# kevalmorabia97/CoVA-Web-Object-Detection

Measured on AMD Instinct MI355X. Metric: webpages/sec fwd+bwd (90 bboxes, K=24), higher is better.
Workload: dtype f32

## Files before the change

cova-web-object-detection_amd/_build.py:

```python
import glob
import os
import subprocess

PKG_DIR = os.path.dirname(os.path.abspath(__file__))
LIB_PATH = os.path.join(PKG_DIR, "lib", "libcova_hip.so")
SOURCES = sorted(glob.glob(os.path.join(PKG_DIR, "csrc", "*.hip")))
HEADERS = sorted(glob.glob(os.path.join(PKG_DIR, "csrc", "*.h")))


def needs_build():
    if not os.path.exists(LIB_PATH):
        return True
    t = os.path.getmtime(LIB_PATH)
    return any(os.path.getmtime(s) > t for s in SOURCES + HEADERS)


FILE_FLAGS = {"conv_wino.hip": ["-fno-slp-vectorize"],
              "conv_wgrad4.hip": ["-fno-slp-vectorize"]}


def build(force=False, verbose=False):
    if not force and not needs_build():
        return LIB_PATH
    hipcc = os.environ.get("HIPCC", "/opt/rocm/bin/hipcc")
    os.makedirs(os.path.dirname(LIB_PATH), exist_ok=True)
    objdir = os.path.join(PKG_DIR, "lib", "obj")
    os.makedirs(objdir, exist_ok=True)
    common = [hipcc, "--offload-arch=gfx950", "-O3", "-std=c++17", "-fPIC", "-fvisibility=hidden",
              "-Wall", "-Wno-unused-function"]
    common += os.environ.get("COVA_EXTRA_FLAGS", "").split()
    if os.environ.get("COVA_ABLATE"):
        common.append("-DCOVA_ABLATE=1")
    procs, objs = [], []
    for src in SOURCES:
        obj = os.path.join(objdir, os.path.basename(src)[:-4] + ".o")
        cmd = common + FILE_FLAGS.get(os.path.basename(src), []) + ["-c", src, "-o", obj]
        if verbose:
            print(" ".join(cmd))
        procs.append((cmd, subprocess.Popen(cmd)))
        objs.append(obj)
    for cmd, p in procs:
        if p.wait() != 0:
            raise subprocess.CalledProcessError(p.returncode, cmd)
    link = [hipcc, "--offload-arch=gfx950", "-shared", "-fPIC"] + objs + ["-o", LIB_PATH]
    if verbose:
        print(" ".join(link))
    subprocess.check_call(link)
    return LIB_PATH


if __name__ == "__main__":
    print(build(force=True, verbose=True))
```

cova-web-object-detection_amd/csrc/conv.hip:

```cpp
#include "common.h"
#include <stdlib.h>
#include "bf3.h"
#include "bn_tail.h"
#include <utility>
#include <type_traits>

namespace {

struct BnBwdEpi {
    const float *act, *z, *mean, *invstd;
};

__device__ __forceinline__ void epilogue_store_stats(const f32x16 &acc0, const f32x16 &acc1,
                                                     float *__restrict__ out,
                                                     const float *__restrict__ addend,
                                                     size_t pix_row_base, int x0, int W,
                                                     bool row_valid, int lane, float &s0,
                                                     float &s1, float &q0, float &q1,
                                                     const BnBwdEpi bn = BnBwdEpi{nullptr, nullptr,
                                                                                  nullptr, nullptr})
{
    const int li = lane & 31;
    s0 = s1 = q0 = q1 = 0.f;
    float mu0 = 0.f, mu1 = 0.f, is0 = 0.f, is1 = 0.f;
// ... 1075 lines not shown
                        const int ph = P0 + k, cph = ph < pool.H2 ? ph : pool.H2 - 1;
#pragma unroll
                        for (int e = 0; e <= par; ++e) {
                            const int pwc = W0 + e, cpw = pwc < pool.W2 ? pwc : pool.W2 - 1;
                            const unsigned o = (unsigned)((cph * pool.W2 + cpw) * 64 + c4 * 4);
                            o_.dpv[par][k][e] = *reinterpret_cast<const f32x4 *>(db + o);
                            o_.cdv[par][k][e] = *reinterpret_cast<const uint32_t *>(ib + o);
                            ok |= (ph < pool.H2 && pwc < pool.W2) ? (1u << (4 + 4 * par + 2 * k + e)) : 0u;
                        }
                    }
                }
            }
            o_.ok = ok;
        };
        auto finish = [&](const Ops &o_, uint32_t *dst) {
            if (WG1R_ABL & 4) return;
            const unsigned ok = o_.ok;
#pragma unroll
            for (int par = 0; par < 2; ++par) {
                const int kx0 = par ? 2 : 1;
                float d[2][4];
#pragma unroll
                for (int rr = 0; rr < 2; ++rr) {
                    float g[4] = {0.f, 0.f, 0.f, 0.f};
                    if (POOL) {
#pragma unroll
                        for (int k = 0; k < 2; ++k) {
                            if (rr == 0 && k == 1) continue;
                            const uint32_t ky = rr == 0 ? 1u : (k == 0 ? 2u : 0u);
#pragma unroll
                            for (int e = 0; e <= par; ++e) {
                                const uint32_t code = ky * 3u + (e == 0 ? (uint32_t)kx0 : 0u);
                                const bool win = (ok >> (4 + 4 * par + 2 * k + e)) & 1u;
#pragma unroll
                                for (int jx = 0; jx < 4; ++jx)
                                    g[jx] += (win && ((o_.cdv[par][k][e] >> (8 * jx)) & 255u) == code) ? o_.dpv[par][k][e][jx] : 0.f;
                            }
                        }
                    }
                    const bool in = (ok >> (2 * par + rr)) & 1u;
#pragma unroll
                    for (int jx = 0; jx < 4; ++jx) {
                        float v = o_.yv[par][rr][jx];
                        if (POOL) v = fmaf(cA[jx], g[jx], fmaf(cB[jx], v, cC[jx]));
                        d[rr][jx] = in ? v : 0.f;
                    }
                }
                u32x4 w0, w1, w2;
#pragma unroll
                for (int jx = 0; jx < 4; ++jx) {
                    uint32_t u0, u1, u2;
                    bf3_split_pair(d[0][jx], d[1][jx], u0, u1, u2);
                    w0[jx] = u0; w1[jx] = u1; w2[jx] = u2;
                }
                u32x4 *o4 = reinterpret_cast<u32x4 *>(dst + ((hp * 16 + cbase + par) * 3) * 64 + c4 * 4);
                o4[0] = w0;
                o4[16] = w1;
                o4[32] = w2;
            }
        };
        if (t0 < ntiles) {
            load_tile(opa, coords(t0));
            finish(opa, s_d);
            load_tile(opb, coords(t0 + tstep));
            load_tile(opc, coords(t0 + 2 * tstep));
        }
        __syncthreads();
        int nb = 1;
        for (int tile = t0; tile < ntiles; tile += 3 * tstep) {
#define WG1R_PSTEP(A_, B_, K_)                                                                   \
            WG1R_STAMP(0);                                                                       \
            finish(A_, s_d + nb * D_DW);                                                         \
            WG1R_STAMP(3);                                                                       \
            load_tile(B_, coords(tile + (K_) * tstep));                                          \
            WG1R_STAMP(1);                                                                       \
            c1b_lds_barrier();                                                                   \
            WG1R_STAMP(2);                                                                       \
            nb ^= 1;                                                                             \
            WG1R_TRIT();
            WG1R_PSTEP(opb, opa, 3)
            if (tile + tstep >= ntiles) break;
            WG1R_PSTEP(opc, opb, 4)
            if (tile + 2 * tstep >= ntiles) break;
            WG1R_PSTEP(opa, opc, 5)
        }
    }
}

__global__ __launch_bounds__(1024) void conv1_wgrad_reduce_kernel(const float *__restrict__ part,
                                                                  int nparts, float *__restrict__ dw)
{
    __shared__ double s_acc[16][64];
    const int tx = threadIdx.x & 63, slice = threadIdx.x >> 6;
    const int idx = blockIdx.x * 64 + tx;
    double s = 0.0;
    for (int p0 = slice; p0 < nparts; p0 += 16 * 8) {
        float v[8];
#pragma unroll
        for (int u = 0; u < 8; ++u) {
            const int p = p0 + 16 * u;
            v[u] = part[(size_t)(p < nparts ? p : p0) * (64 * 160) + idx];
        }
#pragma unroll
        for (int u = 0; u < 8; ++u)
            if (p0 + 16 * u < nparts) s += (double)v[u];
    }
    s_acc[slice][tx] = s;
    __syncthreads();
    if (slice == 0) {
        double t = 0.0;
        for (int j = 0; j < 16; ++j) t += s_acc[j][tx];
        const int co = idx / 160, k = idx - co * 160;
        if (k < 147) dw[co * 147 + k] = (float)t;
    }
}

extern int g_grid_cap;
bool g_options_frozen = false;
inline int persistent_grid(int ntiles, int blocks_per_cu = 1)
{
    g_options_frozen = true;
    static int cus_of[64] = {0};
    int dev = 0;
    if (hipGetDevice(&dev) != hipSuccess || dev < 0 || dev >= 64) dev = 0;
    int cus = cus_of[dev];
    if (cus == 0) {
        hipDeviceProp_t prop;
        if (hipGetDeviceProperties(&prop, dev) == hipSuccess) cus = prop.multiProcessorCount;
        if (cus <= 0) cus = 256;
        cus_of[dev] = cus;
    }
    int g = ntiles < cus * blocks_per_cu ? ntiles : cus * blocks_per_cu;
    if (g_grid_cap > 0 && g > g_grid_cap) g = g_grid_cap;
    return g;
}

int g_ablate = 0;
int g_grid_cap = 0;
int g_conv1_f32 = 0;

}

int cova_internal_persistent_grid(int ntiles) { return persistent_grid(ntiles); }
int cova_internal_persistent_grid2(int ntiles, int blocks_per_cu) { return persistent_grid(ntiles, blocks_per_cu); }

int cova_internal_set_wino4_f32(int v);
int cova_internal_set_bn1d_variant(int v);
int cova_internal_set_gat_wide(int v);
int cova_internal_get_bn1d_variant();
int cova_internal_get_gat_wide();
int cova_internal_get_wino4_f32();
int cova_internal_get_sgemm_dma();
int cova_internal_set_sgemm_dma(int v);
COVA_API int cova_set_option(int key, int value)
{
    static const bool allow = [] { const char *e = getenv("COVA_ALLOW_OPTION_CHANGES"); return e != nullptr && e[0] == '1'; }();
    int cur;
    switch (key) {
    case 2: cur = g_grid_cap; break;
    case 7: cur = g_conv1_f32; value = value != 0; break;
    case 9: cur = cova_internal_get_wino4_f32(); value = value != 0; break;
    case 14: cur = cova_internal_get_bn1d_variant(); break;
    case 16: cur = cova_internal_get_gat_wide(); value = value != 0; break;
    case 22: cur = cova_internal_get_sgemm_dma(); value = value != 0; break;
    default: return COVA_ERR_BAD_ARG;
    }
    if (cur == value) return COVA_OK;
    if (g_options_frozen && !allow) return COVA_ERR_BAD_ARG;
    switch (key) {
    case 2: g_grid_cap = value; return COVA_OK;
    case 7: g_conv1_f32 = value; return COVA_OK;
    case 9: return cova_internal_set_wino4_f32(value);
    case 14: return cova_internal_set_bn1d_variant(value);
    case 22: return cova_internal_set_sgemm_dma(value);
    default: return cova_internal_set_gat_wide(value);
    }
}

#ifdef C1B_TRACE
COVA_API int cova_wg1b_trace_read(unsigned long long *host)
{
    return (int)hipMemcpyFromSymbol(host, HIP_SYMBOL(g_wg1b_trace), sizeof(unsigned long long) * 8 * 20 * 8);
}
COVA_API int cova_c1b_trace_read(unsigned long long *host)
{
    return (int)hipMemcpyFromSymbol(host, HIP_SYMBOL(g_c1b_trace), sizeof(unsigned long long) * 2 * 4 * 20 * 8);
}
#endif

COVA_API int cova_conv_out_size(int in_size, int kernel, int stride, int pad)
{
    return (in_size + 2 * pad - kernel) / stride + 1;
}

COVA_API int cova_conv1_num_tiles(int B, int H, int W);
static int conv1_fwd_tiles(int B, int H, int W)
{
    const int H1 = cova_conv_out_size(H, 7, 2, 3), W1 = cova_conv_out_size(W, 7, 2, 3);
    return g_conv1_f32 ? B * cdiv(H1, c1::TH) * cdiv(W1, c1::TW) : B * cdiv(H1, c1b::TH) * cdiv(W1, c1b::TW);
}

COVA_API int cova_conv1_num_partials(int B, int H, int W)
{
    return persistent_grid(conv1_fwd_tiles(B, H, W), g_conv1_f32 ? 2 : 1);
}

COVA_API int cova_conv1_num_tiles(int B, int H, int W)
{
    const int H1 = cova_conv_out_size(H, 7, 2, 3), W1 = cova_conv_out_size(W, 7, 2, 3);
    return B * cdiv(H1, c1::TH) * cdiv(W1, c1::TW);
}

COVA_API int cova_conv1_prep_weights(const float *w_oihw, float *w_k, void *stream)
{
    COVA_REQUIRE(w_oihw && w_k);
    hipLaunchKernelGGL(prep_w7x7_kernel, dim3(cdiv(c1::W_FLOATS, 256)), dim3(256), 0,
                       (hipStream_t)stream, w_oihw, w_k);
    COVA_LAUNCH_CHECK();
    return COVA_OK;
}

static int conv1_fwd_launch(const float *img, const float *w_k, int w_oihw, float *out, float *stat_part, int B, int H,
                           int W, const cova_bn_tail *tail, void *stream)
{
    COVA_REQUIRE(img && w_k && out && B > 0 && H > 0 && W > 0);
    BnTail t{};
    if (tail != nullptr && tail->mode != 0) {
        t = *tail;
        COVA_REQUIRE(t.mode == 1 && stat_part && t.counter && t.count > 0 && t.gamma && t.beta && t.scale && t.shift &&
                     t.mean && t.invstd);
    }
    const int H1 = cova_conv_out_size(H, 7, 2, 3), W1 = cova_conv_out_size(W, 7, 2, 3);
    if (!g_conv1_f32) {
        const int tiles_x = cdiv(W1, c1b::TW), tiles_y = cdiv(H1, c1b::TH);
        const int ntiles = B * tiles_x * tiles_y;
        const dim3 pgrid(persistent_grid(ntiles, 1)), block(c1b::THREADS);
        if (stat_part)
            hipLaunchKernelGGL(conv1_7x7_bf3_kernel<true>, pgrid, block, 0, (hipStream_t)stream, img, w_k, out, stat_part,
                               H, W, H1, W1, tiles_x, tiles_y, ntiles, w_oihw, t);
        else
            hipLaunchKernelGGL(conv1_7x7_bf3_kernel<false>, pgrid, block, 0, (hipStream_t)stream, img, w_k, out,
                               stat_part, H, W, H1, W1, tiles_x, tiles_y, ntiles, w_oihw, t);
        COVA_LAUNCH_CHECK();
        return COVA_OK;
    }
    const int tiles_x = cdiv(W1, c1::TW), tiles_y = cdiv(H1, c1::TH);
    const dim3 block(c1::THREADS);
    const int ntiles = B * tiles_x * tiles_y;
    const dim3 pgrid(persistent_grid(ntiles, 2));
    if (stat_part)
        hipLaunchKernelGGL(conv1_7x7_v2_kernel<true>, pgrid, block, 0, (hipStream_t)stream, img,
                           w_k, out, stat_part, H, W, H1, W1, tiles_x, tiles_y, ntiles, g_ablate, w_oihw, t);
    else
        hipLaunchKernelGGL(conv1_7x7_v2_kernel<false>, pgrid, block, 0, (hipStream_t)stream, img,
                           w_k, out, stat_part, H, W, H1, W1, tiles_x, tiles_y, ntiles, g_ablate, w_oihw, t);
    COVA_LAUNCH_CHECK();
    return COVA_OK;
}

COVA_API int cova_conv1_fwd(const float *img, const float *w_k, float *out, float *stat_part,
                            int B, int H, int W, void *stream)
{
    return conv1_fwd_launch(img, w_k, 0, out, stat_part, B, H, W, nullptr, stream);
}

COVA_API int cova_conv1_fwd_tail(const float *img, const float *w_oihw, float *out, float *stat_part, int B, int H,
                                 int W, const cova_bn_tail *tail, void *stream)
{
    return conv1_fwd_launch(img, w_oihw, 1, out, stat_part, B, H, W, tail, stream);
}

COVA_API int cova_conv1_wgrad_workspace_floats(int B, int H, int W)
{
    return persistent_grid(cova_conv1_num_tiles(B, H, W)) * 8 * 64 * 160;
}

COVA_API int cova_conv1_wgrad_poolbwd(const float *img, const float *y1, const float *dp,
                                      const uint8_t *idx, const float *abc, float *dw, float *ws,
                                      int B, int H, int W, void *stream)
{
    COVA_REQUIRE(img && y1 && dp && idx && abc && dw && ws && B > 0 && H > 0 && W > 0);
    COVA_REQUIRE((long long)H * W * 64 < (1ll << 31));
    const int H1 = cova_conv_out_size(H, 7, 2, 3), W1 = cova_conv_out_size(W, 7, 2, 3);
    const int H2 = cova_conv_out_size(H1, 3, 2, 1), W2 = cova_conv_out_size(W1, 3, 2, 1);
    const int tiles_x = cdiv(W1, wg1::TW), tiles_y = cdiv(H1, wg1::TH);
    const int grid = persistent_grid(B * tiles_x * tiles_y);
    if (!g_conv1_f32) {
        const int rtx = cdiv(W1, wg1r::TW), rty = cdiv(H1, wg1r::TH);
        const int rgrid = persistent_grid(B * rtx * rty);
        hipLaunchKernelGGL(conv1_wgrad_rs_kernel<true>, dim3(rgrid), dim3(wg1r::THREADS), 0, (hipStream_t)stream, img, y1,
                           ws, H, W, H1, W1, rtx, rty, B * rtx * rty, PoolBwd{dp, idx, abc, H2, W2});
        COVA_LAUNCH_CHECK();
        hipLaunchKernelGGL(conv1_wgrad_reduce_kernel, dim3(64 * 160 / 64), dim3(1024), 0, (hipStream_t)stream, ws,
                           rgrid * 2, dw);
        COVA_LAUNCH_CHECK();
        return COVA_OK;
    }
    hipLaunchKernelGGL(conv1_wgrad_v2_kernel<true>, dim3(grid), dim3(wg1::THREADS), 0,
                       (hipStream_t)stream, img, y1, ws, H, W, H1, W1, tiles_x, tiles_y,
                       B * tiles_x * tiles_y, PoolBwd{dp, idx, abc, H2, W2});
    COVA_LAUNCH_CHECK();
    hipLaunchKernelGGL(conv1_wgrad_reduce_kernel, dim3(64 * 160 / 64), dim3(1024), 0,
                       (hipStream_t)stream, ws, grid * 4, dw);
    COVA_LAUNCH_CHECK();
    return COVA_OK;
}

COVA_API int cova_conv1_wgrad(const float *img, const float *dy, float *dw, float *ws, int B, int H,
                              int W, void *stream)
{
    COVA_REQUIRE(img && dy && dw && ws && B > 0 && H > 0 && W > 0);
    COVA_REQUIRE((long long)H * W * 64 < (1ll << 31));
    const int H1 = cova_conv_out_size(H, 7, 2, 3), W1 = cova_conv_out_size(W, 7, 2, 3);
    const int tiles_x = cdiv(W1, wg1::TW), tiles_y = cdiv(H1, wg1::TH);
    const int grid = persistent_grid(B * tiles_x * tiles_y);
    if (!g_conv1_f32) {
        const int rtx = cdiv(W1, wg1r::TW), rty = cdiv(H1, wg1r::TH);
        const int rgrid = persistent_grid(B * rtx * rty);
        hipLaunchKernelGGL(conv1_wgrad_rs_kernel<false>, dim3(rgrid), dim3(wg1r::THREADS), 0, (hipStream_t)stream, img, dy,
                           ws, H, W, H1, W1, rtx, rty, B * rtx * rty, PoolBwd{nullptr, nullptr, nullptr, 0, 0});
        COVA_LAUNCH_CHECK();
        hipLaunchKernelGGL(conv1_wgrad_reduce_kernel, dim3(64 * 160 / 64), dim3(1024), 0, (hipStream_t)stream, ws,
                           rgrid * 2, dw);
        COVA_LAUNCH_CHECK();
        return COVA_OK;
    }
    hipLaunchKernelGGL(conv1_wgrad_v2_kernel<false>, dim3(grid), dim3(wg1::THREADS), 0,
// ... 9 lines not shown
```

cova-web-object-detection_amd/csrc/conv_wgrad4.hip:

```cpp
#include "common.h"
#include <type_traits>

#ifndef WG4_ABL
#define WG4_ABL 0
#endif

int cova_internal_persistent_grid2(int ntiles, int blocks_per_cu);

#if defined(__HIP_DEVICE_COMPILE__) && !defined(__gfx950__)
#error "conv_wgrad4.hip is written for gfx950 (160 KB of LDS per workgroup)"
#endif

#ifdef WG4_TRACE
__device__ unsigned long long g_wg4_trace[2 * 4 * 8];
#define WG4_STAMP(slot)                                                                                         \
    do {                                                                                                        \
        if (blockIdx.x == 0 && (wave == 0 || wave == 4) && wg4_k >= 100 && wg4_k < 104 && lane == 0)           \
            g_wg4_trace[((wave >> 2) * 4 + (wg4_k - 100)) * 8 + (slot)] = __builtin_amdgcn_s_memtime();         \
    } while (0)
#else
#define WG4_STAMP(slot) do { } while (0)
#endif

namespace {

namespace wg4 {
constexpr int THREADS = 512;
constexpr int ROW = 10;
constexpr int TILE_FLOATS = 128 * ROW + 32;
constexpr int BUF_FLOATS = 2 * 4 * TILE_FLOATS;
constexpr int RAW_FLOATS = 36 * 64;
constexpr int PART_FLOATS = 9 * 4096;
}

struct Wg4Args {
    const float *act, *dz, *dz2;
    float *part;
    const float *act_abc, *dz_abc;
    float *dz_out;
    int act_relu;
    int H, W, tiles_y, strips, nseg_y, seg_rows, nsegs;
};

typedef __attribute__((address_space(3))) void wg4_lds_void;

__device__ __forceinline__ f32x4 wg4_mfma(float a, float b, f32x4 c)
{
    return __builtin_amdgcn_mfma_f32_16x16x4f32(a, b, c, 0, 0, 0);
}

__device__ __forceinline__ void wg4_lds_barrier() { asm volatile("s_waitcnt lgkmcnt(0)\n\ts_barrier" ::: "memory"); }

__device__ __forceinline__ void wg4_copy16(const char *base, unsigned off_bytes, unsigned lds_base_bytes)
{
    asm volatile("s_mov_b32 m0, %0\n\tglobal_load_lds_dwordx4 %1, %2" ::"s"(lds_base_bytes), "v"(off_bytes), "s"(base) : "memory", "m0");
}

__device__ __forceinline__ void wg4_bt6(const float (&d)[6], float (&o)[6])
{
    const float a = fmaf(-4.f, d[2], d[4]), b = fmaf(-4.f, d[1], d[3]);
    const float c = d[4] - d[2], e = 2.f * (d[3] - d[1]);
    o[0] = fmaf(4.f, d[0], fmaf(-5.f, d[2], d[4]));
    o[1] = a + b;
    o[2] = a - b;
    o[3] = c + e;
    o[4] = c - e;
    o[5] = fmaf(4.f, d[1], fmaf(-5.f, d[3], d[5]));
}

__device__ __forceinline__ void wg4_a6(const float (&g)[4], float (&o)[6])
{
    const float p = g[0] + g[2], q = g[1] + g[3];
    const float u = fmaf(4.f, g[2], g[0]), w = 2.f * fmaf(4.f, g[3], g[1]);
    o[0] = g[0];
    o[1] = p + q;
    o[2] = p - q;
    o[3] = u + w;
    o[4] = u - w;
    o[5] = g[3];
}

template <int HALF>
__device__ __forceinline__ void wg4_bt_half(float d0, float d1, float d2, float d3, float d4, float d5, float (&o)[3])
{
    if (HALF == 0) {
        const float a = fmaf(-4.f, d2, d4), b = fmaf(-4.f, d1, d3);
        o[0] = fmaf(4.f, d0, fmaf(-5.f, d2, d4));
        o[1] = a + b;
        o[2] = a - b;
    } else {
        const float c = d4 - d2, e = 2.f * (d3 - d1);
        o[0] = fmaf(4.f, d1, fmaf(-5.f, d3, d5));
        o[1] = c + e;
        o[2] = c - e;
    }
}

template <int HALF>
__device__ __forceinline__ void wg4_a_half(float g0, float g1, float g2, float g3, float (&o)[3])
{
    if (HALF == 0) {
        const float p = g0 + g2, q = g1 + g3;
        o[0] = g0;
        o[1] = p + q;
        o[2] = p - q;
    } else {
        const float u = fmaf(4.f, g2, g0), w = 2.f * fmaf(4.f, g3, g1);
        o[0] = g3;
        o[1] = u + w;
        o[2] = u - w;
    }
}

struct Wg4It {
    int seg, rr, nrows, b, strip, ty;
};

template <bool PROA, int PROD>
__global__ __launch_bounds__(wg4::THREADS, 1) void conv3x3_wgrad4_kernel(const Wg4Args a)
{
    using namespace wg4;
    __shared__ __attribute__((aligned(16))) float s_op[2 * BUF_FLOATS];
    __shared__ __attribute__((aligned(1024))) float s_raw[8 * RAW_FLOATS];
    const int tid = threadIdx.x, lane = tid & 63;
    const int wave = __builtin_amdgcn_readfirstlane(tid >> 6);
    const int H = a.H, W = a.W;
    const int G = (int)gridDim.x, NW = G >> 1;
    int half, walker;
    if ((G & 15) == 0) {
        const int m = (int)blockIdx.x >> 3, x = (int)blockIdx.x & 7;
        half = m & 1;
        walker = (m >> 1) * 8 + x;
    } else {
        half = (int)blockIdx.x & 1;
        walker = (int)blockIdx.x >> 1;
    }
    const bool vrole = wave < 4;
    const int tcol = wave & 3;
    const int pg = wave & 1, cp = (wave >> 1) & 1, np = wave >> 2;
    const int l15 = lane & 15, kq = lane >> 4;

    int n_k = 0;
    for (int s = walker; s < a.nsegs; s += NW) n_k += min(a.seg_rows, a.tiles_y - (s % a.nseg_y) * a.seg_rows);

    auto seg_setup = [&](Wg4It &it) __attribute__((always_inline)) {
        const int s = it.seg < a.nsegs ? it.seg : walker;
        const int sy = s % a.nseg_y, st = (s / a.nseg_y) % a.strips;
        it.b = s / (a.nseg_y * a.strips);
        it.strip = st;
        it.ty = sy * a.seg_rows;
        it.nrows = min(a.seg_rows, a.tiles_y - it.ty);
        it.rr = 0;
    };
    auto advance = [&](Wg4It &it) __attribute__((always_inline)) {
        if (++it.rr < it.nrows) {
            ++it.ty;
        } else {
            it.seg += NW;
            seg_setup(it);
        }
// ... 231 lines not shown
        using Fl = std::false_type;
        using H0 = std::integral_constant<int, 0>;
        using H1 = std::integral_constant<int, 1>;
        if (vrole) {
            if (half == 0) run(T{}, H0{});
            else run(T{}, H1{});
        } else {
            if (half == 0) run(Fl{}, H0{});
            else run(Fl{}, H1{});
        }
    }
    auto fold_values = [&](auto hsel, auto psel, auto esel, float (&tv)[4][9]) __attribute__((always_inline)) {
        constexpr int HALF = decltype(hsel)::value, PG = decltype(psel)::value, e = decltype(esel)::value;
        constexpr double G[6][3] = {{0.25, 0.0, 0.0},         {-1.0 / 6, -1.0 / 6, -1.0 / 6}, {-1.0 / 6, 1.0 / 6, -1.0 / 6},
                                    {1.0 / 24, 1.0 / 12, 1.0 / 6}, {1.0 / 24, -1.0 / 12, 1.0 / 6}, {0.0, 0.0, 1.0}};
        {
            {
#pragma unroll
            for (int r = 0; r < 4; ++r) {
                double T[9];
#pragma unroll
                for (int k = 0; k < 9; ++k) T[k] = 0.0;
#pragma unroll
                for (int al = 0; al < 3; ++al) {
                    constexpr int p0 = 9 * PG, p1 = 9 * PG + 9;
                    if (6 * al + 6 <= p0 || 6 * al >= p1) continue;
                    const int arow = HALF == 0 ? al : (al == 0 ? 5 : 2 + al);
                    double c[3] = {0.0, 0.0, 0.0};
#pragma unroll
                    for (int b = 0; b < 6; ++b) {
                        const int pos = 6 * al + b;
                        if (pos < p0 || pos >= p1) continue;
                        const double qv = (double)acc[pos - p0][e][r];
#pragma unroll
                        for (int t = 0; t < 3; ++t)
                            if (G[b][t] != 0.0) c[t] = fma(G[b][t], qv, c[t]);
                    }
#pragma unroll
                    for (int r3 = 0; r3 < 3; ++r3)
#pragma unroll
                        for (int t = 0; t < 3; ++t)
                            if (G[arow][r3] != 0.0) T[r3 * 3 + t] = fma(G[arow][r3], c[t], T[r3 * 3 + t]);
                }
#pragma unroll
                for (int k = 0; k < 9; ++k) tv[r][k] = (float)T[k];
            }
            }
        }
    };
    float *dst = a.part + (size_t)blockIdx.x * PART_FLOATS;
    auto fold_round = [&](auto esel) __attribute__((always_inline)) {
        constexpr int e = decltype(esel)::value;
        using H0 = std::integral_constant<int, 0>;
        using H1 = std::integral_constant<int, 1>;
        float *xch = s_op + (e & 1) * (4 * 36 * 64) + (wave >> 1) * (36 * 64) + lane;
        float tv[4][9];
        if (half == 0) { if (pg == 0) fold_values(H0{}, H0{}, esel, tv); else fold_values(H0{}, H1{}, esel, tv); }
        else           { if (pg == 0) fold_values(H1{}, H0{}, esel, tv); else fold_values(H1{}, H1{}, esel, tv); }
        if (pg == 1) {
#pragma unroll
            for (int r = 0; r < 4; ++r)
#pragma unroll
                for (int k = 0; k < 9; ++k) xch[(r * 9 + k) * 64] = tv[r][k];
        }
        __syncthreads();
        if (pg == 0) {
            const int i = e >> 1, j = e & 1;
#pragma unroll
            for (int r = 0; r < 4; ++r)
#pragma unroll
                for (int k = 0; k < 9; ++k)
                    dst[k * 4096 + (16 * (2 * cp + i) + 4 * kq + r) * 64 + 16 * (2 * np + j) + l15] =
                        tv[r][k] + xch[(r * 9 + k) * 64];
        }
    };
    __syncthreads();
    fold_round(std::integral_constant<int, 0>{});
    fold_round(std::integral_constant<int, 1>{});
    fold_round(std::integral_constant<int, 2>{});
    fold_round(std::integral_constant<int, 3>{});
}

struct Wg4FinishJobs { const float *part[4]; float *dw[4]; };
__global__ __launch_bounds__(1024) void wgrad4_finish_kernel(const Wg4FinishJobs jobs, int grid)
{
    __shared__ double s_acc[9][16][64];
    const float *__restrict__ part = jobs.part[blockIdx.y];
    float *__restrict__ dw = jobs.dw[blockIdx.y];
    const int tx = threadIdx.x & 63, slice = threadIdx.x >> 6;
    const int idx = blockIdx.x * 64 + tx;
    double acc[9];
#pragma unroll
    for (int k = 0; k < 9; ++k) acc[k] = 0.0;
    for (int blk0 = slice; blk0 < grid; blk0 += 16 * 8) {
        float v[8][9];
#pragma unroll
        for (int u = 0; u < 8; ++u) {
            const int blk = blk0 + 16 * u;
            const float *row = part + (size_t)(blk < grid ? blk : blk0) * wg4::PART_FLOATS + idx;
#pragma unroll
            for (int k = 0; k < 9; ++k) v[u][k] = row[k * 4096];
        }
#pragma unroll
        for (int u = 0; u < 8; ++u)
            if (blk0 + 16 * u < grid) {
#pragma unroll
                for (int k = 0; k < 9; ++k) acc[k] += (double)v[u][k];
            }
    }
#pragma unroll
    for (int k = 0; k < 9; ++k) s_acc[k][slice][tx] = acc[k];
    __syncthreads();
    if (slice < 9) {
        double t = 0.0;
        for (int j = 0; j < 16; ++j) t += s_acc[slice][j][tx];
        dw[idx * 9 + slice] = (float)t;
    }
}

struct Wg4Geo { int tiles_y, strips, nseg_y, seg_rows, nsegs, grid; };

Wg4Geo wg4_geometry(int B, int H, int W)
{
    Wg4Geo g;
    g.tiles_y = cdiv(H, 4);
    g.strips = cdiv(W, 16);
    g.nseg_y = (g.tiles_y + 10) / 20 > 0 ? (g.tiles_y + 10) / 20 : 1;
    g.seg_rows = cdiv(g.tiles_y, g.nseg_y);
    g.nseg_y = cdiv(g.tiles_y, g.seg_rows);
    g.nsegs = B * g.strips * g.nseg_y;
    const int cus = cova_internal_persistent_grid2(1 << 30, 1);
    int walkers = cus / 2 > 0 ? cus / 2 : 1;
    if (walkers > g.nsegs) walkers = g.nsegs;
    g.grid = 2 * walkers;
    return g;
}

int launch_wgrad4(const float *act, const float *act_abc, int act_relu, const float *dz, const float *dz2,
                  const float *dz_abc, float *dz_out, float *ws, int B, int H, int W, hipStream_t st)
{
    const Wg4Geo g = wg4_geometry(B, H, W);
    const Wg4Args a{act, dz, dz_abc ? dz2 : nullptr, ws, act_abc, dz_abc, dz_abc ? dz_out : nullptr, act_relu, H, W,
                    g.tiles_y, g.strips, g.nseg_y, g.seg_rows, g.nsegs};
    const dim3 grid(g.grid), blk(wg4::THREADS);
    const int prod = !dz_abc ? 0 : (dz2 ? 2 : 1);
#define COVA_WG4(PA, PD) hipLaunchKernelGGL((conv3x3_wgrad4_kernel<PA, PD>), grid, blk, 0, st, a)
    if (act_abc) { if (prod == 2) COVA_WG4(true, 2); else if (prod == 1) COVA_WG4(true, 1); else COVA_WG4(true, 0); }
    else         { if (prod == 2) COVA_WG4(false, 2); else if (prod == 1) COVA_WG4(false, 1); else COVA_WG4(false, 0); }
#undef COVA_WG4
    COVA_LAUNCH_CHECK();
    return COVA_OK;
}

}

COVA_API int cova_conv3x3_wgrad4_num_partials(int B, int H, int W) { return wg4_geometry(B, H, W).grid; }

COVA_API int cova_conv3x3_wgrad4_workspace_floats(int B, int H, int W)
{
    const int grid = wg4_geometry(B, H, W).grid;
    return grid * wg4::PART_FLOATS;
}

COVA_API int cova_conv3x3_wgrad4_partial(const float *act, const float *act_abc, int act_relu, const float *dz,
                                         const float *dz2, const float *dz_abc, float *dz_out, float *ws, int B, int H,
                                         int W, void *stream)
{
    COVA_REQUIRE(act && dz && ws && B > 0 && H > 0 && W > 0);
    COVA_REQUIRE((long long)H * W * 256 < (1ll << 32));
    COVA_REQUIRE(dz_out == nullptr || dz_abc != nullptr);
    return launch_wgrad4(act, act_abc, act_relu, dz, dz2, dz_abc, dz_out, ws, B, H, W, (hipStream_t)stream);
}

COVA_API int cova_conv3x3_wgrad4_finish(const float *ws0, float *dw0, const float *ws1, float *dw1, const float *ws2,
                                        float *dw2, const float *ws3, float *dw3, int B, int H, int W, void *stream)
{
    COVA_REQUIRE(B > 0 && H > 0 && W > 0);
    COVA_REQUIRE((ws0 == nullptr) == (dw0 == nullptr) && (ws1 == nullptr) == (dw1 == nullptr) &&
                 (ws2 == nullptr) == (dw2 == nullptr) && (ws3 == nullptr) == (dw3 == nullptr));
    const float *ws[4] = {ws0, ws1, ws2, ws3};
    float *dw[4] = {dw0, dw1, dw2, dw3};
    Wg4FinishJobs jobs{};
    int n = 0;
    for (int i = 0; i < 4; ++i)
        if (ws[i]) { jobs.part[n] = ws[i]; jobs.dw[n] = dw[i]; ++n; }
    if (n == 0) return COVA_OK;
    const int grid = wg4_geometry(B, H, W).grid;
    hipLaunchKernelGGL(wgrad4_finish_kernel, dim3(4096 / 64, n), dim3(1024), 0, (hipStream_t)stream, jobs, grid);
    COVA_LAUNCH_CHECK();
    return COVA_OK;
}

#ifdef WG4_TRACE
COVA_API int cova_wg4_trace_read(unsigned long long *host64)
{
    return (int)hipMemcpyFromSymbol(host64, HIP_SYMBOL(g_wg4_trace), sizeof(unsigned long long) * 64);
}
#endif

COVA_API int cova_conv3x3_wgrad4(const float *act, const float *dz, float *dw, float *ws, int B, int H, int W, void *stream)
{
    COVA_REQUIRE(act && dz && dw && ws && B > 0 && H > 0 && W > 0);
    const int rc = launch_wgrad4(act, nullptr, 0, dz, nullptr, nullptr, nullptr, ws, B, H, W, (hipStream_t)stream);
    if (rc != COVA_OK) return rc;
    return cova_conv3x3_wgrad4_finish(ws, dw, nullptr, nullptr, nullptr, nullptr, nullptr, nullptr, B, H, W, stream);
}
```

Before: 1732.

## Add Winograd F(2,3) bf16x3 MFMA weight-gradient kernel as default wgrad path

```diff
diff --git a/cova-web-object-detection_amd/_build.py b/cova-web-object-detection_amd/_build.py
--- a/cova-web-object-detection_amd/_build.py
+++ b/cova-web-object-detection_amd/_build.py
@@ -15,8 +15,8 @@
     return any(os.path.getmtime(s) > t for s in SOURCES + HEADERS)
 
 
-FILE_FLAGS = {"conv_wino.hip": ["-fno-slp-vectorize"],
-              "conv_wgrad4.hip": ["-fno-slp-vectorize"]}
+FILE_FLAGS = {"conv_wgrad4.hip": ["-fno-slp-vectorize"],
+              "conv_wgrad2s.hip": ["-fno-slp-vectorize"]}
 
 
 def build(force=False, verbose=False):
diff --git a/cova-web-object-detection_amd/csrc/conv.hip b/cova-web-object-detection_amd/csrc/conv.hip
--- a/cova-web-object-detection_amd/csrc/conv.hip
+++ b/cova-web-object-detection_amd/csrc/conv.hip
@@ -1251,6 +1251,8 @@
 int cova_internal_get_wino4_f32();
 int cova_internal_get_sgemm_dma();
 int cova_internal_set_sgemm_dma(int v);
+int cova_internal_get_wgrad_f32();
+int cova_internal_set_wgrad_f32(int v);
 COVA_API int cova_set_option(int key, int value)
 {
     static const bool allow = [] { const char *e = getenv("COVA_ALLOW_OPTION_CHANGES"); return e != nullptr && e[0] == '1'; }();
@@ -1262,6 +1264,7 @@
     case 14: cur = cova_internal_get_bn1d_variant(); break;
     case 16: cur = cova_internal_get_gat_wide(); value = value != 0; break;
     case 22: cur = cova_internal_get_sgemm_dma(); value = value != 0; break;
+    case 23: cur = cova_internal_get_wgrad_f32(); value = value != 0; break;
     default: return COVA_ERR_BAD_ARG;
     }
     if (cur == value) return COVA_OK;
@@ -1272,6 +1275,7 @@
     case 9: return cova_internal_set_wino4_f32(value);
     case 14: return cova_internal_set_bn1d_variant(value);
     case 22: return cova_internal_set_sgemm_dma(value);
+    case 23: return cova_internal_set_wgrad_f32(value);
     default: return cova_internal_set_gat_wide(value);
     }
 }
diff --git a/cova-web-object-detection_amd/csrc/conv_wgrad2s.hip b/cova-web-object-detection_amd/csrc/conv_wgrad2s.hip
--- /dev/null
+++ b/cova-web-object-detection_amd/csrc/conv_wgrad2s.hip
@@ -0,0 +1,408 @@
+#include "bf3.h"
+#include <type_traits>
+
+#ifndef WG2S_ABL
+#define WG2S_ABL 0
+#endif
+#if defined(__HIP_DEVICE_COMPILE__) && !defined(__gfx950__)
+#error "conv_wgrad2s.hip is written for gfx950 (160 KB of LDS per workgroup)"
+#endif
+
+#ifndef WG2S_CHAIN
+#define WG2S_CHAIN 0
+#endif
+
+int cova_internal_persistent_grid2(int ntiles, int blocks_per_cu);
+
+namespace {
+
+namespace wg2 {
+constexpr int THREADS = 512;
+constexpr int STEP_DW = 2 * 4 * 3 * 8 * 64;
+constexpr int STAGE_FLOATS = 28 * 64;
+constexpr int PART_FLOATS = 9 * 4096;
+}
+
+struct Wg2Args {
+    const float *act, *dz, *dz2;
+    float *part;
+    const float *act_abc, *dz_abc;
+    float *dz_out;
+    int act_relu;
+    int H, W, tiles_y, strips, nseg_y, seg_rows, nsegs;
+};
+
+struct Wg2It {
+    int seg, rr, nrows, b, strip, ty;
+};
+
+__device__ __forceinline__ void wg2_lds_barrier() { asm volatile("s_waitcnt lgkmcnt(0)\n\ts_barrier" ::: "memory"); }
+
+typedef __attribute__((address_space(3))) void wg2_lds_void;
+
+__device__ __forceinline__ void wg2_copy16(const char *base, unsigned off_bytes, unsigned lds_base_bytes)
+{
+    asm volatile("s_mov_b32 m0, %0\n\tglobal_load_lds_dwordx4 %1, %2" ::"s"(lds_base_bytes), "v"(off_bytes), "s"(base) : "memory", "m0");
+}
+
+__device__ __forceinline__ f32x16 wg2_mfma(const u32x4 &x, const u32x4 &y, f32x16 c)
+{
+    return __builtin_amdgcn_mfma_f32_32x32x16_bf16(__builtin_bit_cast(bf16x8, x), __builtin_bit_cast(bf16x8, y), c, 0, 0, 0);
+}
+
+template <bool PROA, int PROD>
+__global__ __launch_bounds__(wg2::THREADS, 1) void conv3x3_wgrad2s_kernel(const Wg2Args a)
+{
+    using namespace wg2;
+    __shared__ __attribute__((aligned(16))) uint32_t s_op[2 * STEP_DW];
+    __shared__ __attribute__((aligned(1024))) float s_stage[8 * STAGE_FLOATS];
+    const int tid = threadIdx.x, lane = tid & 63;
+    const int wave = __builtin_amdgcn_readfirstlane(tid >> 6);
+    const int H = a.H, W = a.W, G = (int)gridDim.x;
+    const int jw = wave & 3, coh = wave >> 2;
+    const int r31 = lane & 31, hk = lane >> 5;
+    constexpr bool TWO = PROD == 2;
+
+    int n_k = 0;
+    for (int s = (int)blockIdx.x; s < a.nsegs; s += G) n_k += min(a.seg_rows, a.tiles_y - (s % a.nseg_y) * a.seg_rows);
+
+    auto seg_setup = [&](Wg2It &it) __attribute__((always_inline)) {
+        const int s = it.seg < a.nsegs ? it.seg : (int)blockIdx.x;
+        const int sy = s % a.nseg_y, st = (s / a.nseg_y) % a.strips;
+        it.b = s / (a.nseg_y * a.strips);
+        it.strip = st;
+        it.ty = sy * a.seg_rows;
+        it.nrows = min(a.seg_rows, a.tiles_y - it.ty);
+        it.rr = 0;
+    };
+    auto advance = [&](Wg2It &it) __attribute__((always_inline)) {
+        if (++it.rr < it.nrows) {
+            ++it.ty;
+        } else {
+            it.seg += G;
+            seg_setup(it);
+        }
+    };
+
+    f32x16 acc[4][2];
+#pragma unroll
+    for (int i = 0; i < 4; ++i)
+#pragma unroll
+        for (int n = 0; n < 2; ++n)
+#pragma unroll
+            for (int e = 0; e < 16; ++e) acc[i][n][e] = 0.f;
+
+    const float relu_floor = a.act_relu ? 0.f : -INFINITY;
+    float aA = 1.f, aC = 0.f, gA = 1.f, gB = 0.f, gC = 0.f;
+    if (PROA) { aA = a.act_abc[lane]; aC = a.act_abc[128 + lane]; }
+    if (PROD) { gA = a.dz_abc[lane]; gC = a.dz_abc[128 + lane]; }
+    if (TWO) gB = a.dz_abc[64 + lane];
+    const bool emit = PROD != 0 && a.dz_out != nullptr;
+
+    unsigned lane4 = (unsigned)lane * 4u;
+    asm volatile("" : "+v"(lane4));
+    auto ld = [&](const char *page, int pix) __attribute__((always_inline)) {
+        unsigned ob = (unsigned)pix * 256u;
+        asm volatile("" : "+s"(ob));
+        return *reinterpret_cast<const float *>(page + ob + lane4);
+    };
+    auto page_of = [&](const float *t, const Wg2It &it) __attribute__((always_inline)) {
+        return reinterpret_cast<const char *>(t) + (size_t)it.b * (size_t)H * (size_t)W * 256u;
+    };
+
+    float d[4][6], gd[2][4];
+
+    float *stg = s_stage + wave * STAGE_FLOATS;
+    const unsigned stg_lds = (unsigned)(size_t)(wg2_lds_void *)stg;
+    const float *stg_r = stg + lane;
+    const int sub = lane >> 4, c4 = lane & 15;
+    unsigned in_off[3];
+#pragma unroll
+    for (int q = 0; q < 3; ++q) {
+        const int sl = 4 * q + sub, r = sl >= 6 ? 1 : 0, c = sl - 6 * r;
+        in_off[q] = (unsigned)((r * W + c) * 256 + c4 * 16);
+    }
+    const unsigned g_off = (unsigned)(sub * 256 + c4 * 16);
+    auto request = [&](const Wg2It &it) __attribute__((always_inline)) {
+        if (WG2S_ABL & 2) return;
+        const char *pa = page_of(a.act, it), *pd = page_of(a.dz, it);
+        const char *pz = TWO ? page_of(a.dz2, it) : nullptr;
+        const int gy0 = 2 * it.ty, gx0 = 32 * it.strip + 4 * wave;
+        const bool edge = gy0 + 2 >= H || gx0 - 1 < 0 || gx0 + 4 >= W;
+        asm volatile("s_waitcnt lgkmcnt(0)" ::: "memory");
+        if (!edge) {
+            const unsigned bi = (unsigned)(((gy0 + 1) * W + gx0 - 1) * 256), bg = (unsigned)((gy0 * W + gx0) * 256);
+#pragma unroll
+            for (int q = 0; q < 3; ++q) wg2_copy16(pa + bi, in_off[q], stg_lds + 1024u * q);
+#pragma unroll
+            for (int r = 0; r < 2; ++r) {
+                wg2_copy16(pd + bg + (unsigned)(r * W * 256), g_off, stg_lds + 3072u + 1024u * r);
+                if (TWO) wg2_copy16(pz + bg + (unsigned)(r * W * 256), g_off, stg_lds + 5120u + 1024u * r);
+            }
+        } else {
+#pragma unroll
+            for (int q = 0; q < 3; ++q) {
+                const int sl = 4 * q + sub, r = sl >= 6 ? 1 : 0, c = sl - 6 * r;
+                const int gy = min(gy0 + 1 + r, H - 1), gx = min(max(gx0 - 1 + c, 0), W - 1);
+                wg2_copy16(pa, (unsigned)((gy * W + gx) * 256 + c4 * 16), stg_lds + 1024u * q);
+            }
+#pragma unroll
+            for (int r = 0; r < 2; ++r) {
+                const int gy = min(gy0 + r, H - 1), gx = min(gx0 + sub, W - 1);
+                const unsigned eo = (unsigned)((gy * W + gx) * 256 + c4 * 16);
+                wg2_copy16(pd, eo, stg_lds + 3072u + 1024u * r);
+                if (TWO) wg2_copy16(pz, eo, stg_lds + 5120u + 1024u * r);
+            }
+        }
+    };
+
+    auto form = [&](const Wg2It &it) __attribute__((always_inline)) {
+        const int gy0 = 2 * it.ty, gx0 = 32 * it.strip + 4 * wave;
+        auto actv = [&](float v) __attribute__((always_inline)) {
+            return PROA ? fmaxf(fmaf(aA, v, aC), relu_floor) : v;
+        };
+        if (it.rr == 0) {
+            const char *pa = page_of(a.act, it);
+#pragma unroll
+            for (int r = 0; r < 2; ++r) {
+                const int y = gy0 - 1 + r, gy = min(max(y, 0), H - 1);
+#pragma unroll
+                for (int c = 0; c < 6; ++c) {
+                    const int x = gx0 - 1 + c;
+                    float v = (WG2S_ABL & 2) ? 1.f : ld(pa, gy * W + min(max(x, 0), W - 1));
+                    v = actv(v);
+                    if (!(y >= 0 && y < H && x >= 0 && x < W)) v = 0.f;
+                    d[r][c] = v;
+                }
+            }
+        } else {
+#pragma unroll
+            for (int c = 0; c < 6; ++c) { d[0][c] = d[2][c]; d[1][c] = d[3][c]; }
+        }
+        const bool edge = gy0 + 2 >= H || gx0 - 1 < 0 || gx0 + 4 >= W;
+        asm volatile("s_waitcnt vmcnt(0)" ::: "memory");
+        char *po = emit ? reinterpret_cast<char *>(a.dz_out) + (size_t)it.b * (size_t)H * (size_t)W * 256u : nullptr;
+        auto body = [&](auto edge_t) __attribute__((always_inline)) {
+            constexpr bool EDGE = decltype(edge_t)::value;
+#pragma unroll
+            for (int r = 0; r < 2; ++r)
+#pragma unroll
+                for (int c = 0; c < 6; ++c) {
+                    float v = actv((WG2S_ABL & 2) ? 1.f : stg_r[64 * (r * 6 + c)]);
+                    if (EDGE && !(gy0 + 1 + r < H && gx0 - 1 + c >= 0 && gx0 - 1 + c < W)) v = 0.f;
+                    d[2 + r][c] = v;
+                }
+#pragma unroll
+            for (int r = 0; r < 2; ++r)
+#pragma unroll
+                for (int c = 0; c < 4; ++c) {
+                    float v = (WG2S_ABL & 2) ? 1.f : stg_r[64 * (12 + r * 4 + c)];
+                    if (TWO) v = fmaf(gA, v, fmaf(gB, (WG2S_ABL & 2) ? 1.f : stg_r[64 * (20 + r * 4 + c)], gC));
+                    if (PROD == 1) v = fmaf(gA, v, gC);
+                    const bool valid = !EDGE || (gy0 + r < H && gx0 + c < W);
+                    if (PROD != 0 && emit && valid && !(WG2S_ABL & 2)) {
+                        unsigned ob = (unsigned)((gy0 + r) * W + gx0 + c) * 256u;
+                        asm volatile("" : "+s"(ob));
+                        *reinterpret_cast<float *>(po + ob + lane4) = v;
+                    }
+                    if (!valid) v = 0.f;
+                    gd[r][c] = v;
+                }
+        };
+        if (edge) body(std::true_type{});
+        else body(std::false_type{});
+    };
+
+    auto transform = [&](auto isel, uint32_t *buf) __attribute__((always_inline)) {
+        constexpr int i = decltype(isel)::value;
+        if (WG2S_ABL & 8) return;
+        uint32_t *w = buf + wave * 64 + lane;
+        auto put = [&](int op, int j, float xe, float xo) __attribute__((always_inline)) {
+            uint32_t q0, q1, q2;
+            bf3_split_pair(xe, xo, q0, q1, q2);
+            uint32_t *p = w + (op * 4 + j) * (3 * 8 * 64);
+            p[0] = q0;
+            p[8 * 64] = q1;
+            p[2 * 8 * 64] = q2;
+        };
+        {
+            float s[4];
+#pragma unroll
+            for (int c = 0; c < 4; ++c)
+                s[c] = i == 0 ? gd[0][c] : i == 1 ? gd[0][c] + gd[1][c] : i == 2 ? gd[0][c] - gd[1][c] : gd[1][c];
+            put(0, 0, s[0], s[2]);
+            put(0, 1, s[0] + s[1], s[2] + s[3]);
+            put(0, 2, s[0] - s[1], s[2] - s[3]);
+            put(0, 3, s[1], s[3]);
+        }
+        {
+            float t[6];
+#pragma unroll
+            for (int c = 0; c < 6; ++c)
+                t[c] = i == 0 ? d[0][c] - d[2][c] : i == 1 ? d[1][c] + d[2][c] : i == 2 ? d[2][c] - d[1][c] : d[1][c] - d[3][c];
+            put(1, 0, t[0] - t[2], t[2] - t[4]);
+            put(1, 1, t[1] + t[2], t[3] + t[4]);
+            put(1, 2, t[2] - t[1], t[4] - t[3]);
+            put(1, 3, t[1] - t[3], t[3] - t[5]);
+        }
+    };
+
+    const int a_off = (jw * 3 * 8 + 4 * hk) * 64 + 32 * coh + r31;
+    const int b_off = ((4 + jw) * 3 * 8 + 4 * hk) * 64 + r31;
+    auto frag = [&](const uint32_t *p) __attribute__((always_inline)) {
+        u32x4 v;
+        v[0] = p[0]; v[1] = p[64]; v[2] = p[128]; v[3] = p[192];
+        return v;
+    };
+    u32x4 fa[3], fb[3];
+    if (WG2S_ABL & 16) {
+#pragma unroll
+        for (int q = 0; q < 3; ++q) { fa[q] = frag(s_op + a_off + q * 512); fb[q] = frag(s_op + b_off + q * 512); }
+    }
+    auto products = [&](auto isel, const uint32_t *buf) __attribute__((always_inline)) {
+        constexpr int i = decltype(isel)::value;
+        if (WG2S_ABL & 1) return;
+        if (!(WG2S_ABL & 16)) {
+#pragma unroll
+            for (int q = 0; q < 3; ++q) fa[q] = frag(buf + a_off + q * 512);
+        }
+#pragma unroll
+        for (int n = 0; n < 2; ++n) {
+            if (!(WG2S_ABL & 16)) {
+#pragma unroll
+                for (int q = 0; q < 3; ++q) fb[q] = frag(buf + b_off + 32 * n + q * 512);
+            }
+            f32x16 c;
+            if (WG2S_CHAIN) {
+#pragma unroll
+                for (int e = 0; e < 16; ++e) c[e] = 0.f;
+            } else {
+                c = acc[i][n];
+            }
+            c = wg2_mfma(fa[2], fb[0], c);
+            c = wg2_mfma(fa[1], fb[1], c);
+            c = wg2_mfma(fa[0], fb[2], c);
+            c = wg2_mfma(fa[1], fb[0], c);
+            c = wg2_mfma(fa[0], fb[1], c);
+            c = wg2_mfma(fa[0], fb[0], c);
+            if (WG2S_CHAIN) {
+                acc[i][n] += c;
+                __builtin_amdgcn_sched_barrier(0);
+            } else {
+                acc[i][n] = c;
+            }
+        }
+    };
+
+    auto run = [&](auto first_t) __attribute__((always_inline)) {
+        constexpr bool PFIRST = decltype(first_t)::value;
+        using I0 = std::integral_constant<int, 0>;
+        using I1 = std::integral_constant<int, 1>;
+        using I2 = std::integral_constant<int, 2>;
+        using I3 = std::integral_constant<int, 3>;
+        uint32_t *b0 = s_op, *b1 = s_op + STEP_DW;
+        Wg2It nxt;
+        nxt.seg = (int)blockIdx.x;
+        seg_setup(nxt);
+        request(nxt);
+        form(nxt);
+        advance(nxt);
+        if (n_k > 1) request(nxt);
+        transform(I0{}, b0);
+        wg2_lds_barrier();
+#pragma unroll 1
+        for (int k = 0; k < n_k; ++k) {
+            const bool more = k + 1 < n_k;
+            if (PFIRST) products(I0{}, b0);
+            transform(I1{}, b1);
+            if (!PFIRST) products(I0{}, b0);
+            wg2_lds_barrier();
+            if (PFIRST) products(I1{}, b1);
+            transform(I2{}, b0);
+            if (!PFIRST) products(I1{}, b1);
+            wg2_lds_barrier();
+            if (PFIRST) products(I2{}, b0);
+            transform(I3{}, b1);
+            if (!PFIRST) products(I2{}, b0);
+            wg2_lds_barrier();
+            if (PFIRST) products(I3{}, b1);
+            if (more) {
+                form(nxt);
+                advance(nxt);
+                if (k + 2 < n_k) request(nxt);
+                transform(I0{}, b0);
+            }
+            if (!PFIRST) products(I3{}, b1);
+            wg2_lds_barrier();
+        }
+        asm volatile("s_waitcnt vmcnt(0)" ::: "memory");
+    };
+    if (wave < 4) run(std::true_type{});
+    else run(std::false_type{});
+
+    double *xs = reinterpret_cast<double *>(s_op);
+    float *dst = a.part + (size_t)blockIdx.x * PART_FLOATS;
+    __syncthreads();
+#pragma unroll
+    for (int r3 = 0; r3 < 3; ++r3)
+#pragma unroll
+        for (int n = 0; n < 2; ++n) {
+#pragma unroll
+            for (int e = 0; e < 16; ++e) {
+                const double q0 = (double)acc[0][n][e], q1 = (double)acc[1][n][e], q2 = (double)acc[2][n][e],
+                             q3 = (double)acc[3][n][e];
+                const double p = r3 == 0 ? q0 + 0.5 * q1 + 0.5 * q2 : r3 == 1 ? 0.5 * q1 - 0.5 * q2 : 0.5 * q1 + 0.5 * q2 - q3;
+                xs[(wave * 16 + e) * 64 + lane] = p;
+            }
+            __syncthreads();
+#pragma unroll
+            for (int m = 0; m < 4; ++m) {
+                const int e = 4 * m + jw;
+                const double *x = xs + ((coh * 4) * 16 + e) * 64 + lane;
+                const double p0 = x[0], p1 = x[16 * 64], p2 = x[2 * 16 * 64], p3 = x[3 * 16 * 64];
+                const int co = 32 * coh + mfma32_row(e, lane), ci = 32 * n + r31;
+                float *o = dst + (r3 * 3) * 4096 + co * 64 + ci;
+                o[0] = (float)(p0 + 0.5 * p1 + 0.5 * p2);
+                o[4096] = (float)(0.5 * p1 - 0.5 * p2);
+                o[2 * 4096] = (float)(0.5 * p1 + 0.5 * p2 - p3);
+            }
+            __syncthreads();
+        }
+}
+
+struct Wg2Geo { int tiles_y, strips, nseg_y, seg_rows, nsegs, grid; };
+
+Wg2Geo wg2_geometry(int B, int H, int W)
+{
+    Wg2Geo g;
+    g.tiles_y = cdiv(H, 2);
+    g.strips = cdiv(W, 32);
+    g.nseg_y = (g.tiles_y + 10) / 20 > 0 ? (g.tiles_y + 10) / 20 : 1;
+    g.seg_rows = cdiv(g.tiles_y, g.nseg_y);
+    g.nseg_y = cdiv(g.tiles_y, g.seg_rows);
+    g.nsegs = B * g.strips * g.nseg_y;
+    const int cus = cova_internal_persistent_grid2(1 << 30, 1);
+    g.grid = cus < g.nsegs ? cus : g.nsegs;
+    if (g.grid < 1) g.grid = 1;
+    return g;
+}
+
+}
+
+int cova_internal_wg2s_grid(int B, int H, int W) { return wg2_geometry(B, H, W).grid; }
+
+int cova_internal_wg2s_launch(const float *act, const float *act_abc, int act_relu, const float *dz, const float *dz2,
+                              const float *dz_abc, float *dz_out, float *ws, int B, int H, int W, hipStream_t st)
+{
+    const Wg2Geo g = wg2_geometry(B, H, W);
+    const Wg2Args a{act, dz, dz_abc ? dz2 : nullptr, ws, act_abc, dz_abc, dz_abc ? dz_out : nullptr, act_relu, H, W,
+                    g.tiles_y, g.strips, g.nseg_y, g.seg_rows, g.nsegs};
+    const dim3 grid(g.grid), blk(wg2::THREADS);
+    const int prod = !dz_abc ? 0 : (dz2 ? 2 : 1);
+#define COVA_WG2(PA, PD) hipLaunchKernelGGL((conv3x3_wgrad2s_kernel<PA, PD>), grid, blk, 0, st, a)
+    if (act_abc) { if (prod == 2) COVA_WG2(true, 2); else if (prod == 1) COVA_WG2(true, 1); else COVA_WG2(true, 0); }
+    else         { if (prod == 2) COVA_WG2(false, 2); else if (prod == 1) COVA_WG2(false, 1); else COVA_WG2(false, 0); }
+#undef COVA_WG2
+    COVA_LAUNCH_CHECK();
+    return COVA_OK;
+}
diff --git a/cova-web-object-detection_amd/csrc/conv_wgrad4.hip b/cova-web-object-detection_amd/csrc/conv_wgrad4.hip
--- a/cova-web-object-detection_amd/csrc/conv_wgrad4.hip
+++ b/cova-web-object-detection_amd/csrc/conv_wgrad4.hip
@@ -6,6 +6,9 @@
 #endif
 
 int cova_internal_persistent_grid2(int ntiles, int blocks_per_cu);
+int cova_internal_wg2s_grid(int B, int H, int W);
+int cova_internal_wg2s_launch(const float *act, const float *act_abc, int act_relu, const float *dz, const float *dz2,
+                              const float *dz_abc, float *dz_out, float *ws, int B, int H, int W, hipStream_t st);
 
 #if defined(__HIP_DEVICE_COMPILE__) && !defined(__gfx950__)
 #error "conv_wgrad4.hip is written for gfx950 (160 KB of LDS per workgroup)"
@@ -543,14 +546,20 @@
     return COVA_OK;
 }
 
-}
-
-COVA_API int cova_conv3x3_wgrad4_num_partials(int B, int H, int W) { return wg4_geometry(B, H, W).grid; }
+int g_wgrad_f32 = 0;
+
+int wgrad_grid(int B, int H, int W) { return g_wgrad_f32 ? wg4_geometry(B, H, W).grid : cova_internal_wg2s_grid(B, H, W); }
+
+}
+
+int cova_internal_set_wgrad_f32(int v) { g_wgrad_f32 = v != 0; return COVA_OK; }
+int cova_internal_get_wgrad_f32() { return g_wgrad_f32; }
+
+COVA_API int cova_conv3x3_wgrad4_num_partials(int B, int H, int W) { return wgrad_grid(B, H, W); }
 
 COVA_API int cova_conv3x3_wgrad4_workspace_floats(int B, int H, int W)
 {
-    const int grid = wg4_geometry(B, H, W).grid;
-    return grid * wg4::PART_FLOATS;
+    return wgrad_grid(B, H, W) * wg4::PART_FLOATS;
 }
 
 COVA_API int cova_conv3x3_wgrad4_partial(const float *act, const float *act_abc, int act_relu, const float *dz,
@@ -560,6 +569,8 @@
     COVA_REQUIRE(act && dz && ws && B > 0 && H > 0 && W > 0);
     COVA_REQUIRE((long long)H * W * 256 < (1ll << 32));
     COVA_REQUIRE(dz_out == nullptr || dz_abc != nullptr);
+    if (!g_wgrad_f32)
+        return cova_internal_wg2s_launch(act, act_abc, act_relu, dz, dz2, dz_abc, dz_out, ws, B, H, W, (hipStream_t)stream);
     return launch_wgrad4(act, act_abc, act_relu, dz, dz2, dz_abc, dz_out, ws, B, H, W, (hipStream_t)stream);
 }
 
@@ -576,7 +587,7 @@
     for (int i = 0; i < 4; ++i)
         if (ws[i]) { jobs.part[n] = ws[i]; jobs.dw[n] = dw[i]; ++n; }
     if (n == 0) return COVA_OK;
-    const int grid = wg4_geometry(B, H, W).grid;
+    const int grid = wgrad_grid(B, H, W);
     hipLaunchKernelGGL(wgrad4_finish_kernel, dim3(4096 / 64, n), dim3(1024), 0, (hipStream_t)stream, jobs, grid);
     COVA_LAUNCH_CHECK();
     return COVA_OK;
@@ -592,7 +603,7 @@
 COVA_API int cova_conv3x3_wgrad4(const float *act, const float *dz, float *dw, float *ws, int B, int H, int W, void *stream)
 {
     COVA_REQUIRE(act && dz && dw && ws && B > 0 && H > 0 && W > 0);
-    const int rc = launch_wgrad4(act, nullptr, 0, dz, nullptr, nullptr, nullptr, ws, B, H, W, (hipStream_t)stream);
+    const int rc = cova_conv3x3_wgrad4_partial(act, nullptr, 0, dz, nullptr, nullptr, nullptr, ws, B, H, W, stream);
     if (rc != COVA_OK) return rc;
     return cova_conv3x3_wgrad4_finish(ws, dw, nullptr, nullptr, nullptr, nullptr, nullptr, nullptr, B, H, W, stream);
 }
```

Result: no change. 1730 (-0.1%).
